# MisEty/RTG-SLAM

Measured on AMD Instinct MI355X. Metric: hot_path_units_per_sec, higher is better.
Workload: dtype f32; 1 GPU; `value` counts UNITS, not SLAM frames (the SLAM frame rate by the reference's definition is `slam_frames_per_sec`, from the `slam_sequence` leg of --full).  One UNIT per step = 1 ICP track (3 levels x 5 GN iters, 1200x680, on a second HIP stream) + 1 map-optimisation iteration (raster fwd + masked L1 colour / gated depth loss + attach regulariser + raster bwd + fused Adam) over 1200000 random Gaus; gaussians=1200000, mode=single, parallelism=1 GPU

## Files before the change

include/rtgs_debug.h:

```cpp
#ifndef RTGS_DEBUG_H
#define RTGS_DEBUG_H
#include "rtgs_raster.h"
#ifdef __cplusplus
extern "C" {
#endif

void rtgs_raster_set_counters(void* counters);
void rtgs_raster_set_counters_ctx(rtgs_ctx* ctx, void* counters);

void rtgs_raster_set_profiling(int enable);
void rtgs_raster_set_profiling_ctx(rtgs_ctx* ctx, int enable);

void rtgs_raster_set_near_slice(int mode, int budget_per_tile);
void rtgs_raster_set_near_slice_ctx(rtgs_ctx* ctx, int mode, int budget_per_tile);

void rtgs_raster_force_sort_path(int enable);
void rtgs_raster_force_sort_path_ctx(rtgs_ctx* ctx, int enable);
int rtgs_raster_last_timings(float* ms12_host);
int rtgs_raster_last_timings_ctx(rtgs_ctx* ctx, float* ms12_host);

void rtgs_raster_set_bwd_walk_ctx(rtgs_ctx* ctx, int mode);
void rtgs_raster_set_onepass_ctx(rtgs_ctx* ctx, int on);
void rtgs_raster_set_fused_sort_ctx(rtgs_ctx* ctx, int on);
int rtgs_raster_fused_sort_stats_ctx(rtgs_ctx* ctx, int64_t* out18);
void rtgs_raster_set_tile_gather_ctx(rtgs_ctx* ctx, int mode);
int rtgs_raster_tile_gather_stats_ctx(rtgs_ctx* ctx, int64_t* out6);
void rtgs_raster_set_bwd_debug(int bits);
void rtgs_raster_set_bwd_stamps(void* dev);
void rtgs_raster_set_fwd_stamps(void* dev);
#define RTGS_ICP_STAMP_LAUNCHES 16
#define RTGS_ICP_STAMP_WGS 256
void rtgs_icp_set_stamps(void* dev);
void rtgs_tsdf_set_dense(int on);

#ifdef __cplusplus
}
#endif
#endif
```

rtg_slam_amd/csrc/map_ops.hip:

```cpp
#include "../../include/rtgs_raster.h"
#include <hip/hip_runtime.h>
#include <math.h>
#include <stdint.h>
#include "adam_common.h"
#include "activate_common.h"


namespace rtgs {

__global__ void __launch_bounds__(256) activate8_fwd_kernel(const float4* __restrict__ raw8, int64_t n,
                                                            float* __restrict__ opacity, float* __restrict__ scales,
                                                            float4* __restrict__ rots, float* __restrict__ normal) {
  for (int64_t i = (int64_t)blockIdx.x * blockDim.x + threadIdx.x; i < n; i += (int64_t)gridDim.x * blockDim.x)
    activate8_row_store(raw8[2 * i], raw8[2 * i + 1], i, opacity, scales, rots, normal);
}

__global__ void __launch_bounds__(256) activate8_bwd_kernel(const float4* __restrict__ raw8, int64_t n,
                                                            const float* __restrict__ g_op, const float* __restrict__ g_sc,
                                                            const float4* __restrict__ g_rot, const float* __restrict__ g_nrm,
                                                            const uint8_t* __restrict__ row_state,
                                                            float4* __restrict__ g_raw8) {
  for (int64_t i = (int64_t)blockIdx.x * blockDim.x + threadIdx.x; i < n; i += (int64_t)gridDim.x * blockDim.x) {
    if (row_state) {
      const uint8_t s = row_state[i];
// ... 498 lines not shown
};
template <int V>
__device__ __forceinline__ void load_flags(const uint8_t* __restrict__ rmask, const int32_t* __restrict__ didx, int64_t i, bool (&m)[V],
                                           bool (&hit)[V]) {
  if constexpr (V == 4) {
    const uint32_t mm = rmask ? *reinterpret_cast<const uint32_t*>(rmask + i) : 0x01010101u;
    const int4 d = *reinterpret_cast<const int4*>(didx + i);
    m[0] = (mm & 0xffu) != 0; m[1] = (mm & 0xff00u) != 0; m[2] = (mm & 0xff0000u) != 0; m[3] = (mm & 0xff000000u) != 0;
    hit[0] = d.x != -1; hit[1] = d.y != -1; hit[2] = d.z != -1; hit[3] = d.w != -1;
  } else {
    m[0] = !rmask || rmask[i] != 0;
    hit[0] = didx[i] != -1;
  }
}

template <int V>
__global__ void __launch_bounds__(256) slam_loss_sums_kernel(const float* __restrict__ color, const float* __restrict__ depth,
                                                             const int32_t* __restrict__ didx, const float* __restrict__ gt_c,
                                                             const float* __restrict__ gt_d, const uint8_t* __restrict__ rmask,
                                                             int64_t hw, float depth_thr, float* __restrict__ sums) {
  float s_c = 0.f, s_d = 0.f, s_m = 0.f, s_n = 0.f;
  for (int64_t i = ((int64_t)blockIdx.x * blockDim.x + threadIdx.x) * V; i < hw; i += (int64_t)gridDim.x * blockDim.x * V) {
    bool m[V], hit[V];
    load_flags<V>(rmask, didx, i, m, hit);
    PixVec<V> c0, c1, c2, t0, t1, t2, dp, gd;
    c0.load(color, i); c1.load(color + hw, i); c2.load(color + 2 * hw, i);
    t0.load(gt_c, i); t1.load(gt_c + hw, i); t2.load(gt_c + 2 * hw, i);
    dp.load(depth, i); gd.load(gt_d, i);
#pragma unroll
    for (int k = 0; k < V; ++k) {
      if (!m[k]) continue;
      s_n += 1.f;
      s_c += fabsf(c0.v[k] - t0.v[k]) + fabsf(c1.v[k] - t1.v[k]) + fabsf(c2.v[k] - t2.v[k]);
      const float g = gd.v[k], e = dp.v[k] - g;
      if (hit[k] && g > 0.f && e < depth_thr) { s_d += fabsf(e); s_m += 1.f; }
    }
  }
  s_c = wave_sum_shfl(s_c); s_d = wave_sum_shfl(s_d); s_m = wave_sum_shfl(s_m); s_n = wave_sum_shfl(s_n);
  __shared__ float sh[4][4];
  const int lane = threadIdx.x & 63, w = threadIdx.x >> 6;
  if (lane == 0) { sh[0][w] = s_c; sh[1][w] = s_d; sh[2][w] = s_m; sh[3][w] = s_n; }
  __syncthreads();
  if (threadIdx.x < 4) {
    const float t = sh[threadIdx.x][0] + sh[threadIdx.x][1] + sh[threadIdx.x][2] + sh[threadIdx.x][3];
    unsafeAtomicAdd(&sums[threadIdx.x], t);
  }
}

__device__ __forceinline__ uint32_t sign_code(float d) { return d > 0.f ? 1u : (d < 0.f ? 2u : 0u); }

template <int V>
__global__ void __launch_bounds__(256) slam_loss_sums_signs_kernel(const float* __restrict__ color, const float* __restrict__ depth,
                                                                   const int32_t* __restrict__ didx, const float* __restrict__ gt_c,
                                                                   const float* __restrict__ gt_d, const uint8_t* __restrict__ rmask,
                                                                   int64_t hw, float depth_thr,
                                                                   float* __restrict__ sums, uint8_t* __restrict__ signs) {
  float s_c = 0.f, s_d = 0.f, s_m = 0.f, s_n = 0.f;
  for (int64_t i = ((int64_t)blockIdx.x * blockDim.x + threadIdx.x) * V; i < hw; i += (int64_t)gridDim.x * blockDim.x * V) {
    bool m[V], hit[V];
    load_flags<V>(rmask, didx, i, m, hit);
    PixVec<V> c0, c1, c2, t0, t1, t2, dp, gd;
    c0.load(color, i); c1.load(color + hw, i); c2.load(color + 2 * hw, i);
    t0.load(gt_c, i); t1.load(gt_c + hw, i); t2.load(gt_c + 2 * hw, i);
    dp.load(depth, i); gd.load(gt_d, i);
    uint32_t packed = 0u;
#pragma unroll
    for (int k = 0; k < V; ++k) {
      if (!m[k]) continue;
      const float d0 = c0.v[k] - t0.v[k], d1 = c1.v[k] - t1.v[k], d2 = c2.v[k] - t2.v[k];
      s_n += 1.f;
      s_c += fabsf(d0) + fabsf(d1) + fabsf(d2);
      uint32_t code = sign_code(d0) | (sign_code(d1) << 2) | (sign_code(d2) << 4);
      const float g = gd.v[k], e = dp.v[k] - g;
      if (hit[k] && g > 0.f && e < depth_thr) { s_d += fabsf(e); s_m += 1.f; code |= sign_code(e) << 6; }
      packed |= code << (8 * k);
    }
    if constexpr (V == 4) *reinterpret_cast<uint32_t*>(signs + i) = packed;
    else signs[i] = (uint8_t)packed;
  }
  s_c = wave_sum_shfl(s_c); s_d = wave_sum_shfl(s_d); s_m = wave_sum_shfl(s_m); s_n = wave_sum_shfl(s_n);
  __shared__ float sh[4][4];
  const int lane = threadIdx.x & 63, w = threadIdx.x >> 6;
  if (lane == 0) { sh[0][w] = s_c; sh[1][w] = s_d; sh[2][w] = s_m; sh[3][w] = s_n; }
  __syncthreads();
  if (threadIdx.x < 4) {
    const float t = sh[threadIdx.x][0] + sh[threadIdx.x][1] + sh[threadIdx.x][2] + sh[threadIdx.x][3];
    unsafeAtomicAdd(&sums[threadIdx.x], t);
  }
}

__global__ void slam_loss_values_kernel(const float* __restrict__ sums, float cw, float dw, float* __restrict__ loss4) {
  const float inv_c = 1.f / (3.f * fmaxf(sums[3], 1.f));
  const float inv_m = 1.f / fmaxf(sums[2], 1.f);
  const float lc = sums[0] * inv_c, ld = sums[1] * inv_m;
  loss4[1] = lc; loss4[2] = ld; loss4[3] = 0.f;
  loss4[0] = dw * ld + cw * lc;
}

struct SsimWin { float g[11]; };
constexpr int SS_R = 5, SS_T = 16 + 2 * SS_R;

__global__ void __launch_bounds__(256) ssim_fwd_kernel(const float* __restrict__ x1, const float* __restrict__ x2, int H, int W,
                                                       SsimWin win, float* __restrict__ dmaps, float* __restrict__ sums) {
// ... 144 lines not shown

extern "C" size_t rtgs_slam_loss_signs_offset(int32_t H, int32_t W, int32_t with_ssim) {
  const size_t front = 8 * sizeof(float) + (with_ssim ? (size_t)9 * (size_t)H * (size_t)W * sizeof(float) : 0);
  return (front + 15) & ~(size_t)15;
}
extern "C" size_t rtgs_slam_loss_scratch_bytes(int32_t H, int32_t W, int32_t with_ssim) {
  return rtgs_slam_loss_signs_offset(H, W, with_ssim) + (((size_t)H * (size_t)W + 15) & ~(size_t)15);
}

static void ssim_window(rtgs::SsimWin& win) {
  float gf[11], totf = 0.f;
  for (int i = 0; i < 11; ++i) { gf[i] = (float)exp(-(double)((i - 5) * (i - 5)) / (2.0 * 1.5 * 1.5)); totf += gf[i]; }
  for (int i = 0; i < 11; ++i) win.g[i] = gf[i] / totf;
}

extern "C" int rtgs_slam_loss_sums(const float* color, const float* depth, const int32_t* depth_index, const float* gt_color,
                                   const float* gt_depth, int32_t H, int32_t W, const rtgs_loss_cfg* cfg, void* scratch,
                                   void* stream) {
  if (!color || !depth || !depth_index || !gt_color || !gt_depth || !cfg || !scratch || H <= 0 || W <= 0) return -1;
  hipStream_t st = (hipStream_t)stream;
  const int64_t hw = (int64_t)H * W;
  float* sums = (float*)scratch;
  const bool ssim = cfg->render_mask == nullptr && cfg->ssim_weight != 0.f;
  if (!cfg->sums_zeroed && hipMemsetAsync(sums, 0, 8 * sizeof(float), st) != hipSuccess) return -2;
  int64_t blocks = (hw + 255) / 256;
  if (blocks > 192) blocks = 192;
  if (rtgs::loss_vec4_ok(hw, color, depth, depth_index, gt_color, gt_depth, cfg->render_mask, nullptr, nullptr))
    hipLaunchKernelGGL(rtgs::slam_loss_sums_kernel<4>, dim3((unsigned)blocks), dim3(256), 0, st, color, depth, depth_index,
                       gt_color, gt_depth, cfg->render_mask, hw, cfg->add_depth_thres, sums);
  else
    hipLaunchKernelGGL(rtgs::slam_loss_sums_kernel<1>, dim3((unsigned)blocks), dim3(256), 0, st, color, depth, depth_index,
                       gt_color, gt_depth, cfg->render_mask, hw, cfg->add_depth_thres, sums);
  if (ssim) {
    rtgs::SsimWin win;
    ssim_window(win);
    hipLaunchKernelGGL(rtgs::ssim_fwd_kernel, dim3((W + 15) / 16, (H + 15) / 16), dim3(256), 0, st, color, gt_color, H, W, win,
                       sums + 8, sums);
  }
  return hipGetLastError() == hipSuccess ? 0 : -2;
}

extern "C" int rtgs_slam_loss_values(const rtgs_loss_cfg* cfg, const void* scratch, float* loss_out4, void* stream) {
  if (!cfg || !scratch || !loss_out4 || (cfg->render_mask == nullptr && cfg->ssim_weight != 0.f)) return -1;
  hipLaunchKernelGGL(rtgs::slam_loss_values_kernel, dim3(1), dim3(1), 0, (hipStream_t)stream, (const float*)scratch,
                     cfg->color_weight, cfg->depth_weight, loss_out4);
  return hipGetLastError() == hipSuccess ? 0 : -2;
}
extern "C" int rtgs_slam_loss_sums_signs(const float* color, const float* depth, const int32_t* depth_index,
                                         const float* gt_color, const float* gt_depth, int32_t H, int32_t W,
                                         const rtgs_loss_cfg* cfg, void* scratch, float* loss_out4, void* stream) {
  if (!color || !depth || !depth_index || !gt_color || !gt_depth || !cfg || !scratch || H <= 0 || W <= 0) return -1;
  if (cfg->render_mask == nullptr && cfg->ssim_weight != 0.f) return -1;
  hipStream_t st = (hipStream_t)stream;
  const int64_t hw = (int64_t)H * W;
  float* sums = (float*)scratch;
  uint8_t* signs = (uint8_t*)scratch + rtgs_slam_loss_signs_offset(H, W, cfg->render_mask == nullptr);
  if (!cfg->sums_zeroed && hipMemsetAsync(sums, 0, 8 * sizeof(float), st) != hipSuccess) return -2;
  int64_t blocks = (hw + 255) / 256;
  if (blocks > 192) blocks = 192;
  if (rtgs::loss_vec4_ok(hw, color, depth, depth_index, gt_color, gt_depth, cfg->render_mask, nullptr, nullptr) &&
      ((uintptr_t)signs & 3u) == 0)
    hipLaunchKernelGGL(rtgs::slam_loss_sums_signs_kernel<4>, dim3((unsigned)blocks), dim3(256), 0, st, color, depth, depth_index,
                       gt_color, gt_depth, cfg->render_mask, hw, cfg->add_depth_thres, sums, signs);
  else
    hipLaunchKernelGGL(rtgs::slam_loss_sums_signs_kernel<1>, dim3((unsigned)blocks), dim3(256), 0, st, color, depth, depth_index,
                       gt_color, gt_depth, cfg->render_mask, hw, cfg->add_depth_thres, sums, signs);
  if (loss_out4) return rtgs_slam_loss_values(cfg, scratch, loss_out4, stream);
  return hipGetLastError() == hipSuccess ? 0 : -2;
}

extern "C" int rtgs_slam_loss_grads(const float* color, const float* depth, const int32_t* depth_index, const float* gt_color,
                                    const float* gt_depth, int32_t H, int32_t W, const rtgs_loss_cfg* cfg, void* scratch,
                                    float* loss_out4, float* g_color, float* g_depth, void* stream) {
  if (!color || !depth || !depth_index || !gt_color || !gt_depth || !cfg || !scratch || !loss_out4 || !g_color || !g_depth ||
      H <= 0 || W <= 0)
    return -1;
  hipStream_t st = (hipStream_t)stream;
  const int64_t hw = (int64_t)H * W;
  float* sums = (float*)scratch;
  const bool ssim = cfg->render_mask == nullptr && cfg->ssim_weight != 0.f;
  int64_t blocks = (hw + 255) / 256;
// ... 142 lines not shown
```

rtg_slam_amd/csrc/raster_api.hip:

```cpp
#include "../../include/rtgs_raster.h"
#include "../../include/rtgs_debug.h"
#include "raster_common.h"
#include "raster_launch.h"
#include <vector>

#include <rocprim/device/device_radix_sort.hpp>
#include <rocprim/device/device_scan.hpp>
#include <math.h>
#include <new>
#include <stdlib.h>
#include <string.h>

enum { EV_F0 = 0, EV_PRE, EV_SL_BIN, EV_SL_BLEND, EV_SCAN, EV_BIN0, EV_EMIT, EV_SORT, EV_RANGES, EV_BLEND0, EV_BLEND, EV_B0,
       EV_BWALK, EV_BBLEND, EV_BPRE, EV_N };
struct rtgs_ctx {
  int64_t stats[8] = {0};
  struct Switches {
    int slice_mode = 2;
    int slice_budget = 384;
    int bwd_walk = 0;
    bool onepass = true;
    bool fused_sort = true;
    bool speculation = true;
    bool plain_onepass = true;
    bool cull_cache = true, cull_check = false;
    bool loss_signs = true;
    int tile_gather = 1;
  } sw;
  int64_t gather_stats[4] = {0, 0, 0, 0};
  bool gather_blocked = false;
  int64_t loss_path_stats[2] = {0, 0};
  int64_t slice_stats[4] = {0};
  unsigned long long* counters = nullptr;
  uint32_t last_listed = 0;
  uint32_t* fsort_cls = nullptr;
  int32_t fsort_cap = 0, fsort_tiles = 0;
  bool prof = false;
  bool force_sort_path = false;
  bool ev_init = false;
  hipEvent_t ev[EV_N];
  bool ev_set[EV_N] = {false};
  uint32_t* info_host = nullptr;
// ... 57 lines not shown

static rtgs_ctx* default_ctx() {
  static rtgs_ctx* c = [] {
    rtgs_ctx* n = new rtgs_ctx();
    if (const char* e = getenv("RTGS_NEAR_SLICE")) n->sw.slice_mode = atoi(e);
    if (const char* e = getenv("RTGS_NEAR_SLICE_BUDGET")) { const int b = atoi(e); if (b > 0) n->sw.slice_budget = b; }
    if (const char* e = getenv("RTGS_SPECULATE")) n->sw.speculation = atoi(e) != 0;
    if (const char* e = getenv("RTGS_BIN_ONEPASS")) n->sw.onepass = atoi(e) != 0;
    if (const char* e = getenv("RTGS_FWD_SORT")) n->sw.fused_sort = atoi(e) != 0;
    if (const char* e = getenv("RTGS_PLAIN_ONEPASS")) n->sw.plain_onepass = atoi(e) != 0;
    if (const char* e = getenv("RTGS_BWD_WALK")) { const int m = atoi(e); n->sw.bwd_walk = (m >= 1 && m <= 4) ? m : 0; }
    if (const char* e = getenv("RTGS_CULL_CACHE")) n->sw.cull_cache = atoi(e) != 0;
    if (const char* e = getenv("RTGS_CULL_CACHE_CHECK")) n->sw.cull_check = atoi(e) != 0;
    if (const char* e = getenv("RTGS_LOSS_SIGNS")) n->sw.loss_signs = atoi(e) != 0;
    if (const char* e = getenv("RTGS_TILE_GATHER")) { const int m = atoi(e); n->sw.tile_gather = (m >= 0 && m <= 2) ? m : 1; }
    return n;
  }();
  return c;
}
static inline rtgs_ctx* use(rtgs_ctx* c) { return c ? c : default_ctx(); }

static void prof_mark(rtgs_ctx* c, int which, hipStream_t st) {
  if (!c->prof) return;
  if (!c->ev_init) {
    for (int i = 0; i < EV_N; ++i) (void)hipEventCreate(&c->ev[i]);
    c->ev_init = true;
  }
  (void)hipEventRecord(c->ev[which], st);
  c->ev_set[which] = true;
}
// ... 474 lines not shown
  next_seq(c);
  const uint32_t sl = (uint32_t)G.slice_cap <= SLOTS_MAX ? (uint32_t)G.slice_cap : 0u;
  const uint32_t seg2 = (pl.kind != 1 && c->sw.onepass && ((pl.kind == 2 && G.slice_seg) || (immediate && pl.kind == 0))) ? capL : 0u;
  const bool seg_main = seg2 != 0u;
  const BinLayout B = pl.kind == 1 ? bin_layout(0, ntiles, false, (size_t)sl)
                                   : bin_layout(seg2 ? (int64_t)ntiles * (int64_t)seg2 : (int64_t)capR, ntiles, false, (size_t)capS);
  char* bin = (char*)f.binning_resize(f.binning_user, B.total);
  if (!bin) return RTGS_E_ALLOC;
  c->last_bin = bin;
  BwdInfo* const bwd_info = (BwdInfo*)(f.img + I.bwd_info);
  SplatGrad* const slot_grads = (SplatGrad*)(bin + B.slot_grads);
  if (pl.kind == 1) {
    if ((rc = cull_stage(f, pl.kind, !immediate, fail, BwdInfoInit{bwd_info, slot_grads, sl, sl ? 1u : 0u})) != RTGS_OK) return rc;
    prof_mark(c, EV_PRE, st);
    launch_slice_compact(P, slice_sel(f), (uint32_t*)(f.geom + G.slice_ids), f.slice_ctr + 2, f.tiles_touched, f.offsets,
                         f.slice_ctr + 4, nullptr, 0u, nullptr, st);
    c->spec.gathered = tile_gather_chosen(f, pl);
    if ((rc = slice_pass1(f, fail, c->spec.gathered)) != RTGS_OK) return rc;
    prof_mark(c, EV_BLEND0, st); prof_mark(c, EV_BLEND, st);
    c->hint_slice_lists = true; c->hint_main_lists = false;
    c->slice_stats[0] = 1; c->slice_stats[1] = pl.R1; c->slice_stats[2] = pl.n_fin; c->slice_stats[3] = 0;
  } else {
    unsigned long long* const keys_a = (unsigned long long*)(bin + B.keys_a);
    uint32_t* const vals_b = (uint32_t*)(bin + B.vals_b);
    RasterParams pg = p;
    pg.spec_fail = fail;
    SliceList vl{nullptr, nullptr};
    if (pl.kind == 2) {
      if ((rc = cull_stage(f, pl.kind, !immediate, fail, BwdInfoInit{bwd_info, slot_grads, capS, immediate ? 0u : 1u})) != RTGS_OK)
        return rc;
      prof_mark(c, EV_PRE, st);
// ... 90 lines not shown
    const SliceSel sel1 = slice_sel(f);
    if (!sliced) {
      preprocess_all(f, sort_path ? f.sat : nullptr, true);
      if (!sort_path && want_bwd && (rc = scan_slots(f)) != RTGS_OK) return rc;
    } else {
      launch_preprocess_cull(p, f.means3D, f.scales, f.rotations, f.tiles_touched, f.radii, f.out_radii, f.zero_words, f.zero_n,
                             f.zbin, f.uv, f.slice_hist, st);
    }
    DBG(s, st);
    prof_mark(c, EV_PRE, st);
    if (sliced) {
      launch_slice_hist(P, f.zbin, f.tiles_touched, f.radii, f.slice_hist, f.slice_cover, st);
      const bool ask = f.slice_auto && c->ask_first;
      if (ask) next_seq(c);
      launch_slice_compact(P, sel1, (uint32_t*)(f.geom + G.slice_ids), f.slice_ctr + 2, f.tiles_touched, f.offsets,
                           f.slice_ctr + 4, ask ? f.info_host : nullptr, c->seq, nullptr, st);
      if (ask) {
        if ((rc = wait_published(f)) != RTGS_OK) return rc;
        declined = (int32_t)f.pub[6] < 0;
      }
    }
    if (sliced && declined) {
      vis = SliceList{(const uint32_t*)(f.geom + G.vis_ids), f.slice_ctr + 4};
      launch_visible_compact(P, f.zbin, (uint32_t*)(f.geom + G.vis_ids), f.slice_ctr + 4, f.tiles_touched, f.offsets,
                             f.slice_ctr + 5, nullptr, st);
      shade(f, p, vis, sel1, (size_t)P);
      sliced = false;
      considered = true;
    }
    if (sliced) {
      next_seq(c);
// ... 457 lines not shown
  for (uint32_t v : w) {
    if (v == 0xffffffffu) continue;
    const int cls = (int)(v >> 28);
    const int64_t len = (int64_t)(v & 0x0fffffffu);
    if (cls >= FSORT_CLASSES) continue;
    int64_t* o = out18 + 3 * cls;
    o[1] = o[0] == 0 ? len : (len < o[1] ? len : o[1]);
    o[2] = len > o[2] ? len : o[2];
    ++o[0];
  }
  return RTGS_OK;
}
void rtgs_raster_set_tile_gather_ctx(rtgs_ctx* c, int mode) {
  use(c)->sw.tile_gather = (mode >= 0 && mode <= 2) ? mode : 1; use(c)->plan.valid = false; use(c)->gather_blocked = false;
}
int rtgs_raster_tile_gather_stats_ctx(rtgs_ctx* ctx, int64_t* out6) {
  if (!out6) return RTGS_E_INVALID;
  memcpy(out6, use(ctx)->gather_stats, sizeof(use(ctx)->gather_stats));
  out6[4] = GATHER_CHUNK; out6[5] = GATHER_CAND;
  return RTGS_OK;
}
void rtgs_raster_set_bwd_walk_ctx(rtgs_ctx* c, int mode) { use(c)->sw.bwd_walk = (mode >= 1 && mode <= 4) ? mode : 0; }
void rtgs_raster_set_aux_zero_ctx(rtgs_ctx* ctx, void* eight_words) { use(ctx)->aux_zero = (uint32_t*)eight_words; }
int rtgs_raster_last_buffers_ctx(rtgs_ctx* ctx, void** out3) {
  rtgs_ctx* c = use(ctx);
  if (!out3 || !c->last_geom || !c->last_bin || !c->last_img) return RTGS_E_INVALID;
  out3[0] = c->last_geom; out3[1] = c->last_bin; out3[2] = c->last_img;
  return RTGS_OK;
}
int rtgs_raster_backward_buffers(int32_t P, int32_t H, int32_t W, size_t* out) {
// ... 80 lines not shown
```

rtg_slam_amd/csrc/raster_bin.hip:

```cpp
#include "raster_common.h"
#include "raster_launch.h"
#include "raster_tilesort.h"
#include <mutex>

namespace rtgs {

struct LdsGrant {
  std::mutex m;
  size_t got[64];
  explicit LdsGrant(size_t base) { for (size_t& g : got) g = base; }
  void ensure(const void* fn, size_t lds) {
    int dev = 0;
    (void)hipGetDevice(&dev);
    if (dev < 0 || dev >= 64) { (void)hipFuncSetAttribute(fn, hipFuncAttributeMaxDynamicSharedMemorySize, (int)lds); return; }
    std::lock_guard<std::mutex> lk(m);
    if (lds > got[dev]) {
      (void)hipFuncSetAttribute(fn, hipFuncAttributeMaxDynamicSharedMemorySize, (int)lds);
      got[dev] = lds;
    }
  }
};

constexpr int GPB = 1024;
#ifndef RTGS_SLICE_GPB
// ... 478 lines not shown
#pragma unroll
    for (int off = 1; off < 64; off <<= 1) {
      const uint32_t t = (uint32_t)__shfl_up((int)incl, off);
      if (lane >= off) incl += t;
    }
    if (lane == 63) s_w[w] = incl;
    __syncthreads();
    uint32_t pre = s_run;
    for (int q = 0; q < w; ++q) pre += s_w[q];
    if (k < n) { gbase[id] = s_gb + pre + incl - a; ids[s_base + k] = id; }
    __syncthreads();
    if (threadIdx.x == 0) s_run += (s_w[0] + s_w[1]) + (s_w[2] + s_w[3]);
    __syncthreads();
  }
}
void launch_slice_compact(int P, SliceSel sel, uint32_t* ids, uint32_t* n_list, const uint32_t* rect_area, uint32_t* gbase,
                          uint32_t* slot_cursor, uint32_t* host, uint32_t seq, uint32_t* fail_if_taken, hipStream_t st) {
  if (P == 0) return;
  hipLaunchKernelGGL(slice_compact_kernel, dim3((P + COMPACT_CHUNK - 1) / COMPACT_CHUNK), dim3(256), 0, st, P, sel, ids,
                     n_list, rect_area, gbase, slot_cursor, host, seq, fail_if_taken);
}

constexpr int VIS_CHUNK = 8192;
__global__ void __launch_bounds__(256) visible_compact_kernel(int P, int chunk, const uint8_t* __restrict__ zbin, uint32_t* __restrict__ ids,
                                                              uint32_t* __restrict__ n_list,
                                                              const uint32_t* __restrict__ rect_area,
                                                              uint32_t* __restrict__ gbase, uint32_t* __restrict__ slot_cursor,
                                                              const uint32_t* __restrict__ spec_fail, SliceSel sel,
                                                              int32_t* __restrict__ cut_out, uint32_t* __restrict__ fail_if_taken) {
  __shared__ uint32_t s_ids[VIS_CHUNK];
  if (spec_failed(spec_fail)) return;
  if (cut_out) {
    const int cut = slice_cut(sel);
    if (blockIdx.x == 0 && threadIdx.x == 0) {
      *cut_out = cut;
// ... 161 lines not shown
```

rtg_slam_amd/csrc/raster_launch.h:

```cpp
#pragma once
#include "raster_common.h"

namespace rtgs {

void set_fwd_stamps(void* dev);
void launch_mask_sat(const int32_t* mask, int gx, int gy, int32_t* sat, hipStream_t st);
void launch_preprocess_fwd(const RasterParams& p, const float* means, const float* opac, const float* shs, const float* scales,
                           const float* rots, const float* normal_w, const int32_t* sat, Splat* splats, uint32_t* tiles_touched,
                           int32_t* radii, uint8_t* clamped, int32_t* out_radii, uint32_t* zero_words, int zero_n, uint8_t* zbin,
                           hipStream_t st);
void launch_preprocess_cull(const RasterParams& p, const float* means, const float* scales, const float* rots,
                            uint32_t* tiles_touched, int32_t* radii, int32_t* out_radii, uint32_t* zero_words, int zero_n,
                            uint8_t* zbin, float2* uv, uint32_t* hist_words, hipStream_t st);
void launch_preprocess_shade(const RasterParams& p, const float* means, const float* opac, const float* shs, const float* scales,
                             const float* rots, const float* normal_w, Splat* splats, int32_t* radii, uint8_t* clamped, float2* uv,
                             SliceList list, SliceSel sel, size_t max_items, hipStream_t st,
                             RowBands rb = RowBands{nullptr, nullptr, 0u});
void launch_recull_rows(const RasterParams& p, const float* means, const float* scales, const float* rots, uint32_t* tiles_touched,
                        int32_t* radii, int32_t* out_radii, uint32_t* zero_words, int zero_n, uint8_t* zbin, float2* uv,
                        uint32_t* hist, unsigned long long* cover, uint8_t* marks, const float* view_copy, int fail_idx,
                        BwdInfoInit bi, hipStream_t st);
void launch_cull_check(int P, const uint32_t* tt_a, const uint32_t* tt_b, const int32_t* rad_a, const int32_t* rad_b,
                       const int32_t* orad_a, const int32_t* orad_b, const uint8_t* zb_a, const uint8_t* zb_b, const float2* uv_a,
                       const float2* uv_b, const uint32_t* hist_a, const uint32_t* hist_b, const uint32_t* skip,
// ... 29 lines not shown
void launch_blend_bwd_entry(const RasterParams& p, const uint2* ranges, const uint32_t* point_list, const Splat* splats,
                            const float* out_color, const uint32_t* n_contrib, const int32_t* depth_index,
                            const uint32_t* depth_pos, const uint32_t* tile_last, const float* dL_dcolor, const float* dL_ddepth,
                            const uint32_t* gbase, uint32_t* slot_count, const BwdInfo* info, SplatGrad* grads, uint8_t* touched,
                            const uint32_t* tile_mode, uint32_t t0, uint32_t tn, TileCache tc, uint32_t pre, hipStream_t st,
                            const LossSigns* signs = nullptr);

size_t bin_lds_limit_tiles();
int bin_sort_capacity();
size_t bin_block_counts_bytes(int P, int ntiles);
size_t bin_slice_block_counts_bytes(int P, size_t max_list, int ntiles);
size_t bin_list_block_counts_bytes(int P, int ntiles);
void launch_slice_hist(int P, const uint8_t* zbin, const uint32_t* rect_area, const int32_t* radii, uint32_t* hist,
                       unsigned long long* cover, hipStream_t st, BwdInfoInit bi = BwdInfoInit{nullptr, nullptr, 0u, 0u});
void launch_slice_compact(int P, SliceSel sel, uint32_t* ids, uint32_t* n_list, const uint32_t* rect_area, uint32_t* gbase,
                          uint32_t* slot_cursor, uint32_t* host, uint32_t seq, uint32_t* fail_if_taken, hipStream_t st);
void launch_visible_compact(int P, const uint8_t* zbin, uint32_t* ids, uint32_t* n_list, const uint32_t* rect_area,
                            uint32_t* gbase, uint32_t* slot_cursor, const uint32_t* spec_fail, hipStream_t st,
                            const SliceSel* decide = nullptr, int32_t* cut_out = nullptr, uint32_t* fail_if_taken = nullptr);
int launch_bin_count(const RasterParams& p, const Splat* splats, const int32_t* radii, const int32_t* mask, uint32_t* tile_count,
                     uint16_t* block_counts, SliceSel sel, SliceList list, size_t max_items, hipStream_t st);
void launch_bin_tilescan(int ntiles, const uint32_t* tile_count, uint2* ranges, uint32_t* cursor, uint32_t* info,
                         uint32_t* info_host, const uint32_t* extra_src, const uint32_t* extra_src2, const uint32_t* slot_a,
                         const uint32_t* slot_b, uint32_t seq, SpecCaps caps, hipStream_t st);
void launch_bin_scatter(const RasterParams& p, const Splat* splats, const int32_t* radii, const int32_t* mask,
                        const uint16_t* block_counts, uint32_t* cursor, unsigned long long* bucket, SliceSel sel, SliceList list,
                        size_t max_items, hipStream_t st);
void launch_bin_place(const RasterParams& p, const Splat* splats, const int32_t* radii, const int32_t* mask, uint32_t* seg_count,
                      unsigned long long* bucket, uint32_t seg, uint32_t* fail, SliceSel sel, SliceList list, size_t max_items,
                      hipStream_t st);
void launch_bin_tilesort(int ntiles, uint32_t longest, const uint2* ranges, const unsigned long long* bucket, uint32_t* point_list,
// ... 7 lines not shown
```

rtg_slam_amd/rasterizer.py:

```python
from __future__ import annotations

import ctypes as C
import threading
from typing import NamedTuple, Optional

import torch
import torch.nn as nn

from . import _lib


class GaussianRasterizationSettings(NamedTuple):
    image_height: int
    image_width: int
    tanfovx: float
    tanfovy: float
    bg: torch.Tensor
    scale_modifier: float
    viewmatrix: torch.Tensor
    projmatrix: torch.Tensor
    sh_degree: int
    campos: torch.Tensor
    opaque_threshold: float
    depth_threshold: float
# ... 48 lines not shown

    def fused_sort_stats(self):
        out = (C.c_int64 * 18)()
        _lib.check(_lib.load().rtgs_raster_fused_sort_stats_ctx(self.ptr, out), "rtgs_raster_fused_sort_stats")
        names = ("empty", "single", "bitonic", "radix", "launch", "pass2")
        return {n: dict(tiles=int(out[3 * k]), shortest=int(out[3 * k + 1]), longest=int(out[3 * k + 2])) for k, n in enumerate(names)}

    def set_tile_gather(self, mode: int):
        _lib.load().rtgs_raster_set_tile_gather_ctx(self.ptr, int(mode))

    def tile_gather_stats(self):
        out = (C.c_int64 * 6)()
        _lib.check(_lib.load().rtgs_raster_tile_gather_stats_ctx(self.ptr, out), "rtgs_raster_tile_gather_stats")
        return dict(gathered=int(out[0]), fell_back_listed=int(out[1]), fell_back_longest=int(out[2]), fell_back_layout=int(out[3]),
                    chunk=int(out[4]), capacity=int(out[5]))

    def set_loss_signs(self, enable: bool):
        _lib.load().rtgs_raster_set_loss_signs_ctx(self.ptr, int(bool(enable)))

    def loss_signs_stats(self):
        out = (C.c_int64 * 2)()
        _lib.check(_lib.load().rtgs_raster_loss_signs_stats_ctx(self.ptr, out), "rtgs_raster_loss_signs_stats")
        return dict(signs=int(out[0]), floats=int(out[1]))

    def set_speculation(self, enable: bool):
        _lib.load().rtgs_raster_set_speculation_ctx(self.ptr, int(bool(enable)))

    def speculation_stats(self):
        out = (C.c_int64 * 3)()
        _lib.check(_lib.load().rtgs_raster_speculation_stats_ctx(self.ptr, out), "rtgs_raster_speculation_stats")
# ... 308 lines not shown
```

Measured before the change: 3104 units/s.

## Widen loss-sum kernel to 1024-thread blocks and add scan-based slice compaction

```diff
diff --git a/include/rtgs_debug.h b/include/rtgs_debug.h
--- a/include/rtgs_debug.h
+++ b/include/rtgs_debug.h
@@ -25,6 +25,10 @@
 int rtgs_raster_fused_sort_stats_ctx(rtgs_ctx* ctx, int64_t* out18);
 void rtgs_raster_set_tile_gather_ctx(rtgs_ctx* ctx, int mode);
 int rtgs_raster_tile_gather_stats_ctx(rtgs_ctx* ctx, int64_t* out6);
+void rtgs_raster_set_slice_compact_ctx(rtgs_ctx* ctx, int form);
+int rtgs_raster_debug_slice_compact(int32_t P, const uint8_t* zbin, const uint32_t* hist, const uint32_t* rect_area,
+                                    uint32_t cap, uint32_t max_list, uint32_t* ids, uint32_t* ctr8, uint32_t* gbase, int32_t form,
+                                    void* stream);
 void rtgs_raster_set_bwd_debug(int bits);
 void rtgs_raster_set_bwd_stamps(void* dev);
 void rtgs_raster_set_fwd_stamps(void* dev);
@@ -32,6 +36,7 @@
 #define RTGS_ICP_STAMP_WGS 256
 void rtgs_icp_set_stamps(void* dev);
 void rtgs_tsdf_set_dense(int on);
+void rtgs_slam_loss_set_wide(int on);
 
 #ifdef __cplusplus
 }
diff --git a/rtg_slam_amd/csrc/map_ops.hip b/rtg_slam_amd/csrc/map_ops.hip
--- a/rtg_slam_amd/csrc/map_ops.hip
+++ b/rtg_slam_amd/csrc/map_ops.hip
@@ -1,7 +1,9 @@
 #include "../../include/rtgs_raster.h"
+#include "../../include/rtgs_debug.h"
 #include <hip/hip_runtime.h>
 #include <math.h>
 #include <stdint.h>
+#include <stdlib.h>
 #include "adam_common.h"
 #include "activate_common.h"
 
@@ -536,79 +538,83 @@
   }
 }
 
-template <int V>
-__global__ void __launch_bounds__(256) slam_loss_sums_kernel(const float* __restrict__ color, const float* __restrict__ depth,
-                                                             const int32_t* __restrict__ didx, const float* __restrict__ gt_c,
-                                                             const float* __restrict__ gt_d, const uint8_t* __restrict__ rmask,
-                                                             int64_t hw, float depth_thr, float* __restrict__ sums) {
-  float s_c = 0.f, s_d = 0.f, s_m = 0.f, s_n = 0.f;
-  for (int64_t i = ((int64_t)blockIdx.x * blockDim.x + threadIdx.x) * V; i < hw; i += (int64_t)gridDim.x * blockDim.x * V) {
-    bool m[V], hit[V];
-    load_flags<V>(rmask, didx, i, m, hit);
-    PixVec<V> c0, c1, c2, t0, t1, t2, dp, gd;
-    c0.load(color, i); c1.load(color + hw, i); c2.load(color + 2 * hw, i);
-    t0.load(gt_c, i); t1.load(gt_c + hw, i); t2.load(gt_c + 2 * hw, i);
-    dp.load(depth, i); gd.load(gt_d, i);
-#pragma unroll
-    for (int k = 0; k < V; ++k) {
-      if (!m[k]) continue;
-      s_n += 1.f;
-      s_c += fabsf(c0.v[k] - t0.v[k]) + fabsf(c1.v[k] - t1.v[k]) + fabsf(c2.v[k] - t2.v[k]);
-      const float g = gd.v[k], e = dp.v[k] - g;
-      if (hit[k] && g > 0.f && e < depth_thr) { s_d += fabsf(e); s_m += 1.f; }
-    }
-  }
+template <int NW>
+__device__ __forceinline__ void loss_sums_reduce(float s_c, float s_d, float s_m, float s_n, float* __restrict__ sums) {
   s_c = wave_sum_shfl(s_c); s_d = wave_sum_shfl(s_d); s_m = wave_sum_shfl(s_m); s_n = wave_sum_shfl(s_n);
-  __shared__ float sh[4][4];
+  __shared__ float sh[4][NW];
   const int lane = threadIdx.x & 63, w = threadIdx.x >> 6;
   if (lane == 0) { sh[0][w] = s_c; sh[1][w] = s_d; sh[2][w] = s_m; sh[3][w] = s_n; }
   __syncthreads();
   if (threadIdx.x < 4) {
-    const float t = sh[threadIdx.x][0] + sh[threadIdx.x][1] + sh[threadIdx.x][2] + sh[threadIdx.x][3];
+    float t = sh[threadIdx.x][0];
+#pragma unroll
+    for (int q = 1; q < NW; ++q) t += sh[threadIdx.x][q];
     unsafeAtomicAdd(&sums[threadIdx.x], t);
   }
 }
 
-__device__ __forceinline__ uint32_t sign_code(float d) { return d > 0.f ? 1u : (d < 0.f ? 2u : 0u); }
-
-template <int V>
-__global__ void __launch_bounds__(256) slam_loss_sums_signs_kernel(const float* __restrict__ color, const float* __restrict__ depth,
-                                                                   const int32_t* __restrict__ didx, const float* __restrict__ gt_c,
-                                                                   const float* __restrict__ gt_d, const uint8_t* __restrict__ rmask,
-                                                                   int64_t hw, float depth_thr,
-                                                                   float* __restrict__ sums, uint8_t* __restrict__ signs) {
-  float s_c = 0.f, s_d = 0.f, s_m = 0.f, s_n = 0.f;
-  for (int64_t i = ((int64_t)blockIdx.x * blockDim.x + threadIdx.x) * V; i < hw; i += (int64_t)gridDim.x * blockDim.x * V) {
-    bool m[V], hit[V];
+template <int V> struct LossPix {
+  bool m[V], hit[V];
+  PixVec<V> c0, c1, c2, t0, t1, t2, dp, gd;
+  __device__ __forceinline__ void load(const float* __restrict__ color, const float* __restrict__ depth, const int32_t* __restrict__ didx,
+                                       const float* __restrict__ gt_c, const float* __restrict__ gt_d, const uint8_t* __restrict__ rmask,
+                                       int64_t hw, int64_t i) {
     load_flags<V>(rmask, didx, i, m, hit);
-    PixVec<V> c0, c1, c2, t0, t1, t2, dp, gd;
     c0.load(color, i); c1.load(color + hw, i); c2.load(color + 2 * hw, i);
     t0.load(gt_c, i); t1.load(gt_c + hw, i); t2.load(gt_c + 2 * hw, i);
     dp.load(depth, i); gd.load(gt_d, i);
-    uint32_t packed = 0u;
-#pragma unroll
-    for (int k = 0; k < V; ++k) {
-      if (!m[k]) continue;
-      const float d0 = c0.v[k] - t0.v[k], d1 = c1.v[k] - t1.v[k], d2 = c2.v[k] - t2.v[k];
-      s_n += 1.f;
-      s_c += fabsf(d0) + fabsf(d1) + fabsf(d2);
-      uint32_t code = sign_code(d0) | (sign_code(d1) << 2) | (sign_code(d2) << 4);
-      const float g = gd.v[k], e = dp.v[k] - g;
-      if (hit[k] && g > 0.f && e < depth_thr) { s_d += fabsf(e); s_m += 1.f; code |= sign_code(e) << 6; }
-      packed |= code << (8 * k);
-    }
-    if constexpr (V == 4) *reinterpret_cast<uint32_t*>(signs + i) = packed;
-    else signs[i] = (uint8_t)packed;
-  }
-  s_c = wave_sum_shfl(s_c); s_d = wave_sum_shfl(s_d); s_m = wave_sum_shfl(s_m); s_n = wave_sum_shfl(s_n);
-  __shared__ float sh[4][4];
-  const int lane = threadIdx.x & 63, w = threadIdx.x >> 6;
-  if (lane == 0) { sh[0][w] = s_c; sh[1][w] = s_d; sh[2][w] = s_m; sh[3][w] = s_n; }
-  __syncthreads();
-  if (threadIdx.x < 4) {
-    const float t = sh[threadIdx.x][0] + sh[threadIdx.x][1] + sh[threadIdx.x][2] + sh[threadIdx.x][3];
-    unsafeAtomicAdd(&sums[threadIdx.x], t);
-  }
+  }
+};
+__device__ __forceinline__ uint32_t sign_code(float d) { return d > 0.f ? 1u : (d < 0.f ? 2u : 0u); }
+template <int V, bool SIGNS>
+__device__ __forceinline__ uint32_t loss_pix_sums(const LossPix<V>& x, float depth_thr, float& s_c, float& s_d, float& s_m, float& s_n) {
+  uint32_t packed = 0u;
+#pragma unroll
+  for (int k = 0; k < V; ++k) {
+    if (!x.m[k]) continue;
+    const float d0 = x.c0.v[k] - x.t0.v[k], d1 = x.c1.v[k] - x.t1.v[k], d2 = x.c2.v[k] - x.t2.v[k];
+    s_n += 1.f;
+    s_c += fabsf(d0) + fabsf(d1) + fabsf(d2);
+    uint32_t code = SIGNS ? sign_code(d0) | (sign_code(d1) << 2) | (sign_code(d2) << 4) : 0u;
+    const float g = x.gd.v[k], e = x.dp.v[k] - g;
+    if (x.hit[k] && g > 0.f && e < depth_thr) { s_d += fabsf(e); s_m += 1.f; if (SIGNS) code |= sign_code(e) << 6; }
+    packed |= code << (8 * k);
+  }
+  return packed;
+}
+
+template <int V, int THREADS, bool SIGNS>
+__device__ __forceinline__ void loss_sums_body(const float* __restrict__ color, const float* __restrict__ depth,
+                                               const int32_t* __restrict__ didx, const float* __restrict__ gt_c,
+                                               const float* __restrict__ gt_d, const uint8_t* __restrict__ rmask, int64_t hw,
+                                               float depth_thr, float* __restrict__ sums, uint8_t* __restrict__ signs) {
+  float s_c = 0.f, s_d = 0.f, s_m = 0.f, s_n = 0.f;
+  for (int64_t i = ((int64_t)blockIdx.x * THREADS + threadIdx.x) * V; i < hw; i += (int64_t)gridDim.x * THREADS * V) {
+    LossPix<V> x;
+    x.load(color, depth, didx, gt_c, gt_d, rmask, hw, i);
+    const uint32_t packed = loss_pix_sums<V, SIGNS>(x, depth_thr, s_c, s_d, s_m, s_n);
+    if constexpr (SIGNS) {
+      if constexpr (V == 4) *reinterpret_cast<uint32_t*>(signs + i) = packed;
+      else signs[i] = (uint8_t)packed;
+    }
+  }
+  loss_sums_reduce<THREADS / 64>(s_c, s_d, s_m, s_n, sums);
+}
+
+template <int V, int THREADS>
+__global__ void __launch_bounds__(THREADS) slam_loss_sums_kernel(const float* __restrict__ color, const float* __restrict__ depth,
+                                                                 const int32_t* __restrict__ didx, const float* __restrict__ gt_c,
+                                                                 const float* __restrict__ gt_d, const uint8_t* __restrict__ rmask,
+                                                                 int64_t hw, float depth_thr, float* __restrict__ sums) {
+  loss_sums_body<V, THREADS, false>(color, depth, didx, gt_c, gt_d, rmask, hw, depth_thr, sums, nullptr);
+}
+template <int V, int THREADS>
+__global__ void __launch_bounds__(THREADS) slam_loss_sums_signs_kernel(const float* __restrict__ color, const float* __restrict__ depth,
+                                                                       const int32_t* __restrict__ didx, const float* __restrict__ gt_c,
+                                                                       const float* __restrict__ gt_d, const uint8_t* __restrict__ rmask,
+                                                                       int64_t hw, float depth_thr,
+                                                                       float* __restrict__ sums, uint8_t* __restrict__ signs) {
+  loss_sums_body<V, THREADS, true>(color, depth, didx, gt_c, gt_d, rmask, hw, depth_thr, sums, signs);
 }
 
 __global__ void slam_loss_values_kernel(const float* __restrict__ sums, float cw, float dw, float* __restrict__ loss4) {
@@ -783,6 +789,15 @@
   for (int i = 0; i < 11; ++i) win.g[i] = gf[i] / totf;
 }
 
+struct LossGrid { unsigned blocks, threads; };
+static int g_loss_wide = [] { const char* e = getenv("RTGS_LOSS_WIDE"); return e ? (atoi(e) != 0 ? 1 : 0) : 1; }();
+extern "C" void rtgs_slam_loss_set_wide(int on) { g_loss_wide = on != 0 ? 1 : 0; }
+static LossGrid loss_grid(int64_t hw, int V) {
+  if (!g_loss_wide) { const int64_t b = (hw + 255) / 256; return LossGrid{(unsigned)(b > 192 ? 192 : b), 256u}; }
+  const int64_t per = 1024 * V, b = (hw + per - 1) / per;
+  return LossGrid{(unsigned)(b > 200 ? 200 : b), 1024u};
+}
+
 extern "C" int rtgs_slam_loss_sums(const float* color, const float* depth, const int32_t* depth_index, const float* gt_color,
                                    const float* gt_depth, int32_t H, int32_t W, const rtgs_loss_cfg* cfg, void* scratch,
                                    void* stream) {
@@ -792,14 +807,14 @@
   float* sums = (float*)scratch;
   const bool ssim = cfg->render_mask == nullptr && cfg->ssim_weight != 0.f;
   if (!cfg->sums_zeroed && hipMemsetAsync(sums, 0, 8 * sizeof(float), st) != hipSuccess) return -2;
-  int64_t blocks = (hw + 255) / 256;
-  if (blocks > 192) blocks = 192;
-  if (rtgs::loss_vec4_ok(hw, color, depth, depth_index, gt_color, gt_depth, cfg->render_mask, nullptr, nullptr))
-    hipLaunchKernelGGL(rtgs::slam_loss_sums_kernel<4>, dim3((unsigned)blocks), dim3(256), 0, st, color, depth, depth_index,
-                       gt_color, gt_depth, cfg->render_mask, hw, cfg->add_depth_thres, sums);
-  else
-    hipLaunchKernelGGL(rtgs::slam_loss_sums_kernel<1>, dim3((unsigned)blocks), dim3(256), 0, st, color, depth, depth_index,
-                       gt_color, gt_depth, cfg->render_mask, hw, cfg->add_depth_thres, sums);
+  const bool v4 = rtgs::loss_vec4_ok(hw, color, depth, depth_index, gt_color, gt_depth, cfg->render_mask, nullptr, nullptr);
+  const LossGrid lg = loss_grid(hw, v4 ? 4 : 1);
+#define RTGS_LOSS_SUMS(V, T)                                                                                                    \
+  hipLaunchKernelGGL((rtgs::slam_loss_sums_kernel<V, T>), dim3(lg.blocks), dim3(T), 0, st, color, depth, depth_index, gt_color, \
+                     gt_depth, cfg->render_mask, hw, cfg->add_depth_thres, sums)
+  if (lg.threads == 1024) { if (v4) RTGS_LOSS_SUMS(4, 1024); else RTGS_LOSS_SUMS(1, 1024); }
+  else                    { if (v4) RTGS_LOSS_SUMS(4, 256); else RTGS_LOSS_SUMS(1, 256); }
+#undef RTGS_LOSS_SUMS
   if (ssim) {
     rtgs::SsimWin win;
     ssim_window(win);
@@ -825,15 +840,15 @@
   float* sums = (float*)scratch;
   uint8_t* signs = (uint8_t*)scratch + rtgs_slam_loss_signs_offset(H, W, cfg->render_mask == nullptr);
   if (!cfg->sums_zeroed && hipMemsetAsync(sums, 0, 8 * sizeof(float), st) != hipSuccess) return -2;
-  int64_t blocks = (hw + 255) / 256;
-  if (blocks > 192) blocks = 192;
-  if (rtgs::loss_vec4_ok(hw, color, depth, depth_index, gt_color, gt_depth, cfg->render_mask, nullptr, nullptr) &&
-      ((uintptr_t)signs & 3u) == 0)
-    hipLaunchKernelGGL(rtgs::slam_loss_sums_signs_kernel<4>, dim3((unsigned)blocks), dim3(256), 0, st, color, depth, depth_index,
-                       gt_color, gt_depth, cfg->render_mask, hw, cfg->add_depth_thres, sums, signs);
-  else
-    hipLaunchKernelGGL(rtgs::slam_loss_sums_signs_kernel<1>, dim3((unsigned)blocks), dim3(256), 0, st, color, depth, depth_index,
-                       gt_color, gt_depth, cfg->render_mask, hw, cfg->add_depth_thres, sums, signs);
+  const bool v4 = rtgs::loss_vec4_ok(hw, color, depth, depth_index, gt_color, gt_depth, cfg->render_mask, nullptr, nullptr) &&
+                  ((uintptr_t)signs & 3u) == 0;
+  const LossGrid lg = loss_grid(hw, v4 ? 4 : 1);
+#define RTGS_LOSS_SIGNS(V, T)                                                                                              \
+  hipLaunchKernelGGL((rtgs::slam_loss_sums_signs_kernel<V, T>), dim3(lg.blocks), dim3(T), 0, st, color, depth, depth_index, \
+                     gt_color, gt_depth, cfg->render_mask, hw, cfg->add_depth_thres, sums, signs)
+  if (lg.threads == 1024) { if (v4) RTGS_LOSS_SIGNS(4, 1024); else RTGS_LOSS_SIGNS(1, 1024); }
+  else                    { if (v4) RTGS_LOSS_SIGNS(4, 256); else RTGS_LOSS_SIGNS(1, 256); }
+#undef RTGS_LOSS_SIGNS
   if (loss_out4) return rtgs_slam_loss_values(cfg, scratch, loss_out4, stream);
   return hipGetLastError() == hipSuccess ? 0 : -2;
 }
diff --git a/rtg_slam_amd/csrc/raster_api.hip b/rtg_slam_amd/csrc/raster_api.hip
--- a/rtg_slam_amd/csrc/raster_api.hip
+++ b/rtg_slam_amd/csrc/raster_api.hip
@@ -26,6 +26,7 @@
     bool cull_cache = true, cull_check = false;
     bool loss_signs = true;
     int tile_gather = 1;
+    int slice_compact = 1;
   } sw;
   int64_t gather_stats[4] = {0, 0, 0, 0};
   bool gather_blocked = false;
@@ -113,6 +114,7 @@
     if (const char* e = getenv("RTGS_CULL_CACHE_CHECK")) n->sw.cull_check = atoi(e) != 0;
     if (const char* e = getenv("RTGS_LOSS_SIGNS")) n->sw.loss_signs = atoi(e) != 0;
     if (const char* e = getenv("RTGS_TILE_GATHER")) { const int m = atoi(e); n->sw.tile_gather = (m >= 0 && m <= 2) ? m : 1; }
+    if (const char* e = getenv("RTGS_SLICE_COMPACT")) { const int m = atoi(e); n->sw.slice_compact = m != 0 ? 1 : 0; }
     return n;
   }();
   return c;
@@ -617,7 +619,7 @@
     if ((rc = cull_stage(f, pl.kind, !immediate, fail, BwdInfoInit{bwd_info, slot_grads, sl, sl ? 1u : 0u})) != RTGS_OK) return rc;
     prof_mark(c, EV_PRE, st);
     launch_slice_compact(P, slice_sel(f), (uint32_t*)(f.geom + G.slice_ids), f.slice_ctr + 2, f.tiles_touched, f.offsets,
-                         f.slice_ctr + 4, nullptr, 0u, nullptr, st);
+                         f.slice_ctr + 4, nullptr, 0u, nullptr, st, c->sw.slice_compact);
     c->spec.gathered = tile_gather_chosen(f, pl);
     if ((rc = slice_pass1(f, fail, c->spec.gathered)) != RTGS_OK) return rc;
     prof_mark(c, EV_BLEND0, st); prof_mark(c, EV_BLEND, st);
@@ -738,7 +740,7 @@
       const bool ask = f.slice_auto && c->ask_first;
       if (ask) next_seq(c);
       launch_slice_compact(P, sel1, (uint32_t*)(f.geom + G.slice_ids), f.slice_ctr + 2, f.tiles_touched, f.offsets,
-                           f.slice_ctr + 4, ask ? f.info_host : nullptr, c->seq, nullptr, st);
+                           f.slice_ctr + 4, ask ? f.info_host : nullptr, c->seq, nullptr, st, c->sw.slice_compact);
       if (ask) {
         if ((rc = wait_published(f)) != RTGS_OK) return rc;
         declined = (int32_t)f.pub[6] < 0;
@@ -1226,6 +1228,15 @@
 void rtgs_raster_set_tile_gather_ctx(rtgs_ctx* c, int mode) {
   use(c)->sw.tile_gather = (mode >= 0 && mode <= 2) ? mode : 1; use(c)->plan.valid = false; use(c)->gather_blocked = false;
 }
+void rtgs_raster_set_slice_compact_ctx(rtgs_ctx* c, int form) { use(c)->sw.slice_compact = form != 0 ? 1 : 0; }
+int rtgs_raster_debug_slice_compact(int32_t P, const uint8_t* zbin, const uint32_t* hist, const uint32_t* rect_area,
+                                    uint32_t cap, uint32_t max_list, uint32_t* ids, uint32_t* ctr8, uint32_t* gbase, int32_t form,
+                                    void* stream) {
+  if (P < 0 || form < 0 || form > 1 || !hist || !ctr8 || (P > 0 && (!zbin || !rect_area || !ids || !gbase))) return RTGS_E_INVALID;
+  const SliceSel sel{1, zbin, hist, cap, max_list, ctr8, nullptr, nullptr, nullptr, 0u, 0};
+  launch_slice_compact(P, sel, ids, ctr8 + 2, rect_area, gbase, ctr8 + 4, nullptr, 0u, nullptr, (hipStream_t)stream, form);
+  return hipGetLastError() == hipSuccess ? RTGS_OK : RTGS_E_HIP;
+}
 int rtgs_raster_tile_gather_stats_ctx(rtgs_ctx* ctx, int64_t* out6) {
   if (!out6) return RTGS_E_INVALID;
   memcpy(out6, use(ctx)->gather_stats, sizeof(use(ctx)->gather_stats));
diff --git a/rtg_slam_amd/csrc/raster_bin.hip b/rtg_slam_amd/csrc/raster_bin.hip
--- a/rtg_slam_amd/csrc/raster_bin.hip
+++ b/rtg_slam_amd/csrc/raster_bin.hip
@@ -516,11 +516,101 @@
     __syncthreads();
   }
 }
+__global__ void __launch_bounds__(256) slice_compact_scan_kernel(int P, SliceSel sel, uint32_t* __restrict__ ids,
+                                                                 uint32_t* __restrict__ n_list,
+                                                                 const uint32_t* __restrict__ rect_area,
+                                                                 uint32_t* __restrict__ gbase, uint32_t* __restrict__ slot_cursor,
+                                                                 uint32_t* __restrict__ host, uint32_t seq,
+                                                                 uint32_t* __restrict__ fail_if_taken) {
+  constexpr int CHUNK = COMPACT_CHUNK, WORDS = CHUNK / 1024;
+  __shared__ uint32_t s_ids[CHUNK], s_pre[CHUNK];
+  __shared__ uint32_t s_cnt[4], s_area[4], s_base, s_gb;
+  const int lane = threadIdx.x & 63, w = threadIdx.x >> 6;
+  const int begin = blockIdx.x * CHUNK;
+  uint32_t zall[WORDS];
+#pragma unroll
+  for (int j = 0; j < WORDS; ++j) {
+    const int i = begin + j * 1024 + (int)threadIdx.x * 4;
+    uint32_t zb4 = 0xffffffffu;
+    if (i + 4 <= P) zb4 = *reinterpret_cast<const uint32_t*>(sel.zbin + i);
+    else for (int k = 0; k < 4; ++k) if (i + k < P) zb4 = (zb4 & ~(0xffu << (8 * k))) | ((uint32_t)sel.zbin[i + k] << (8 * k));
+    zall[j] = zb4;
+  }
+  const int cut = slice_cut(sel);
+  if (blockIdx.x == 0 && threadIdx.x == 0) {
+    reinterpret_cast<int32_t*>(n_list)[1] = cut;
+    if (fail_if_taken && cut >= 0) *fail_if_taken = 1u;
+    if (host) {
+      const uint32_t hw[7] = {0u, 0u, 0u, 0u, 0u, 0u, (uint32_t)cut};
+      publish_to_host(host, hw, seq);
+    }
+  }
+  uint32_t cnt = 0;
+#pragma unroll
+  for (int j = 0; j < WORDS; ++j)
+#pragma unroll
+    for (int k = 0; k < 4; ++k) {
+      const int zb = (int)((zall[j] >> (8 * k)) & 0xffu);
+      cnt += (zb != 255 && zb <= cut) ? 1u : 0u;
+    }
+  uint32_t incl = cnt;
+#pragma unroll
+  for (int off = 1; off < 64; off <<= 1) {
+    const uint32_t t = (uint32_t)__shfl_up((int)incl, off);
+    if (lane >= off) incl += t;
+  }
+  if (lane == 63) s_cnt[w] = incl;
+  __syncthreads();
+  const uint32_t n = (s_cnt[0] + s_cnt[1]) + (s_cnt[2] + s_cnt[3]);
+  if (n == 0u) return;
+  uint32_t pos = incl - cnt;
+  for (int q = 0; q < w; ++q) pos += s_cnt[q];
+#pragma unroll
+  for (int j = 0; j < WORDS; ++j)
+#pragma unroll
+    for (int k = 0; k < 4; ++k) {
+      const int zb = (int)((zall[j] >> (8 * k)) & 0xffu);
+      if (zb != 255 && zb <= cut) s_ids[pos++] = (uint32_t)(begin + j * 1024 + (int)threadIdx.x * 4 + k);
+    }
+  __syncthreads();
+  const uint32_t q = ((n + 255u) / 256u) * 64u, k_lo = (uint32_t)w * q + (uint32_t)lane;
+  const uint32_t k_end = min(n, (uint32_t)(w + 1) * q);
+#pragma unroll 4
+  for (uint32_t k = k_lo; k < k_end; k += 64u) s_pre[k] = rect_area[s_ids[k]];
+  uint32_t run = 0;
+  for (uint32_t k0 = (uint32_t)w * q; k0 < k_end; k0 += 64u) {
+    const uint32_t k = k0 + (uint32_t)lane;
+    const uint32_t a = k < k_end ? s_pre[k] : 0u;
+    uint32_t in_w = a;
+#pragma unroll
+    for (int off = 1; off < 64; off <<= 1) {
+      const uint32_t t = (uint32_t)__shfl_up((int)in_w, off);
+      if (lane >= off) in_w += t;
+    }
+    if (k < k_end) s_pre[k] = run + in_w - a;
+    run += (uint32_t)__shfl((int)in_w, 63);
+  }
+  if (lane == 0) s_area[w] = run;
+  __syncthreads();
+  if (threadIdx.x == 0) {
+    s_base = atomicAdd(n_list, n);
+    s_gb = atomicAdd(slot_cursor, (s_area[0] + s_area[1]) + (s_area[2] + s_area[3]));
+  }
+  __syncthreads();
+  uint32_t gb = s_gb;
+  for (int p = 0; p < w; ++p) gb += s_area[p];
+  const uint32_t base = s_base;
+  for (uint32_t k = k_lo; k < k_end; k += 64u) {
+    const uint32_t id = s_ids[k];
+    gbase[id] = gb + s_pre[k];
+    ids[base + k] = id;
+  }
+}
 void launch_slice_compact(int P, SliceSel sel, uint32_t* ids, uint32_t* n_list, const uint32_t* rect_area, uint32_t* gbase,
-                          uint32_t* slot_cursor, uint32_t* host, uint32_t seq, uint32_t* fail_if_taken, hipStream_t st) {
+                          uint32_t* slot_cursor, uint32_t* host, uint32_t seq, uint32_t* fail_if_taken, hipStream_t st, int form) {
   if (P == 0) return;
-  hipLaunchKernelGGL(slice_compact_kernel, dim3((P + COMPACT_CHUNK - 1) / COMPACT_CHUNK), dim3(256), 0, st, P, sel, ids,
-                     n_list, rect_area, gbase, slot_cursor, host, seq, fail_if_taken);
+  hipLaunchKernelGGL(form != 0 ? slice_compact_scan_kernel : slice_compact_kernel, dim3((P + COMPACT_CHUNK - 1) / COMPACT_CHUNK),
+                     dim3(256), 0, st, P, sel, ids, n_list, rect_area, gbase, slot_cursor, host, seq, fail_if_taken);
 }
 
 constexpr int VIS_CHUNK = 8192;
diff --git a/rtg_slam_amd/csrc/raster_launch.h b/rtg_slam_amd/csrc/raster_launch.h
--- a/rtg_slam_amd/csrc/raster_launch.h
+++ b/rtg_slam_amd/csrc/raster_launch.h
@@ -67,7 +67,7 @@
 void launch_slice_hist(int P, const uint8_t* zbin, const uint32_t* rect_area, const int32_t* radii, uint32_t* hist,
                        unsigned long long* cover, hipStream_t st, BwdInfoInit bi = BwdInfoInit{nullptr, nullptr, 0u, 0u});
 void launch_slice_compact(int P, SliceSel sel, uint32_t* ids, uint32_t* n_list, const uint32_t* rect_area, uint32_t* gbase,
-                          uint32_t* slot_cursor, uint32_t* host, uint32_t seq, uint32_t* fail_if_taken, hipStream_t st);
+                          uint32_t* slot_cursor, uint32_t* host, uint32_t seq, uint32_t* fail_if_taken, hipStream_t st, int form);
 void launch_visible_compact(int P, const uint8_t* zbin, uint32_t* ids, uint32_t* n_list, const uint32_t* rect_area,
                             uint32_t* gbase, uint32_t* slot_cursor, const uint32_t* spec_fail, hipStream_t st,
                             const SliceSel* decide = nullptr, int32_t* cut_out = nullptr, uint32_t* fail_if_taken = nullptr);
diff --git a/rtg_slam_amd/rasterizer.py b/rtg_slam_amd/rasterizer.py
--- a/rtg_slam_amd/rasterizer.py
+++ b/rtg_slam_amd/rasterizer.py
@@ -86,6 +86,9 @@
         _lib.check(_lib.load().rtgs_raster_tile_gather_stats_ctx(self.ptr, out), "rtgs_raster_tile_gather_stats")
         return dict(gathered=int(out[0]), fell_back_listed=int(out[1]), fell_back_longest=int(out[2]), fell_back_layout=int(out[3]),
                     chunk=int(out[4]), capacity=int(out[5]))
+
+    def set_slice_compact(self, scan: bool):
+        _lib.load().rtgs_raster_set_slice_compact_ctx(self.ptr, int(bool(scan)))
 
     def set_loss_signs(self, enable: bool):
         _lib.load().rtgs_raster_set_loss_signs_ctx(self.ptr, int(bool(enable)))
```

Result: no change. 3099 units/s (-0.2%).
